# qhy991/llama.cpp-quant-gemm

Measured on NVIDIA B200. Metric: q4_0_q8_1_decode_gemv_hbm_gbs, higher is better.
Workload: dtype u4 x s8 -> s32 (dp4a), fp32 fold

## Files before the change

### llama.cpp-quant-gemm_b200/csrc/gemv.cu

```cuda
#include <cstdlib>

#include "ptx.cuh"
#include "qgemm_common.cuh"

namespace qgemm {

constexpr int kGemvWarps = 8;
constexpr int kGemvThreads = (kGemvWarps + 1) * 32;
constexpr int kGemvMaxStages = 8;
constexpr int kGemvInflightTarget = 56 * 1024;
constexpr int kGemvSlotsOff = 128;
constexpr int kGemvAbarOff = kGemvSlotsOff + 2 * kGemvWarps * 8 * 4;
constexpr int kGemvActOff = (kGemvAbarOff + 8 + 127) / 128 * 128;
static_assert(2 * kGemvMaxStages * 8 <= kGemvSlotsOff, "ring barriers overlap the slots");
static_assert(kGemvAbarOff % 8 == 0 && kGemvAbarOff + 8 <= kGemvActOff, "abar must not overlap the bulk-copy destination");
constexpr int kGemvSmemBudget = 110 * 1024;
constexpr int kGemvCtasPerSm = 2;
constexpr int kGemvMaxGroup = 8;
constexpr int kGemvTileTarget = 24 * 1024;

template <int WT> struct Pair { static constexpr int words = Fmt<WT>::bytes / 2; };

template <int WT>
__device__ __forceinline__ void load_pair(const uint8_t* p, uint32_t (&x)[Pair<WT>::words]) {
    if constexpr (WT == QGEMM_TYPE_Q5_1) {
        const uint4* q = reinterpret_cast<const uint4*>(p);
#pragma unroll
        for (int i = 0; i < 3; i++) {
            const uint4 v = q[i];
            x[4 * i] = v.x; x[4 * i + 1] = v.y; x[4 * i + 2] = v.z; x[4 * i + 3] = v.w;
        }
    } else if constexpr (WT == QGEMM_TYPE_Q4_1) {
        const uint2* q = reinterpret_cast<const uint2*>(p);
#pragma unroll
        for (int i = 0; i < 5; i++) {
            const uint2 v = q[i];
            x[2 * i] = v.x; x[2 * i + 1] = v.y;
        }
    } else {
        const uint32_t* q = reinterpret_cast<const uint32_t*>(p);
#pragma unroll
        for (int i = 0; i < Pair<WT>::words; i++) x[i] = q[i];
    }
}

__device__ __forceinline__ void expand4(const uint32_t (&q)[4], uint32_t (&w)[8]) {
#pragma unroll
    for (int i = 0; i < 4; i++) {
        w[i] = q[i] & 0x0f0f0f0fu;
        w[i + 4] = q[i] & 0xf0f0f0f0u;
    }
}
// ... 40 lines not shown
        ws[0] = {half_bits_to_float(x[0]), 0.f};
        ws[1] = {half_bits_to_float(x[5] >> 16), 0.f};
        const uint32_t q0[4] = {fs(x[1], x[2]), fs(x[2], x[3]), fs(x[3], x[4]), fs(x[4], x[5])};
        const uint32_t q1[4] = {x[7], x[8], x[9], x[10]};
        expand5(q0, fs(x[0], x[1]), w[0]);
        expand5(q1, x[6], w[1]);
    } else if constexpr (WT == QGEMM_TYPE_Q5_1) {
        ws[0] = {half_bits_to_float(x[0]), half_bits_to_float(x[0] >> 16)};
        ws[1] = {half_bits_to_float(x[6]), half_bits_to_float(x[6] >> 16)};
        const uint32_t q0[4] = {x[2], x[3], x[4], x[5]};
        const uint32_t q1[4] = {x[8], x[9], x[10], x[11]};
        expand5(q0, x[1], w[0]);
        expand5(q1, x[7], w[1]);
    } else {
        ws[0] = {half_bits_to_float(x[0]), 0.f};
        ws[1] = {half_bits_to_float(x[8] >> 16), 0.f};
#pragma unroll
        for (int i = 0; i < 8; i++) {
            w[0][i] = fs(x[i], x[i + 1]);
            w[1][i] = x[9 + i];
        }
    }
}

struct ActPair {
    int q[2][8];
    ActScale s[2];
};

struct GemvParams {
    const uint8_t* act;
    const uint8_t* wgt;
    float* C;
    int F, nb;
    int64_t ldc_t, ldc_f;
    int RT;
    int WPR;
    int stages;
    int stage_bytes;
    int pdl;
    int nocompute;
    int act_bulk;
    PeerOut peer;
    const uint8_t* pf_ptr;
    unsigned long long pf_bytes;
    int nmat;
    const uint8_t* wgt_m[kGemvMaxGroup];
    float* C_m[kGemvMaxGroup];
    int fstart[kGemvMaxGroup + 1];
    float skew;
#ifdef QGEMM_GEMV_TRACE
    int trace_slot;
#endif
};

#ifdef QGEMM_GEMV_TRACE
constexpr int kTraceSlots = 256, kTraceCtas = 304;
__device__ unsigned long long g_gemv_trace[kTraceSlots][kTraceCtas][6];
__device__ __forceinline__ unsigned long long gtimer() {
    unsigned long long t;
    asm volatile("mov.u64 %0, %%globaltimer;" : "=l"(t));
    return t;
}
#define GEMV_TRACE(i) do { if (threadIdx.x == 0 && blockIdx.x < kTraceCtas) g_gemv_trace[p.trace_slot][blockIdx.x][i] = gtimer(); } while (0)
#else
#define GEMV_TRACE(i)
#endif

struct TileRef { int m, local, rows; };
__device__ __forceinline__ TileRef tile_at(const GemvParams& p, int r0, int r_end) {
    TileRef t{0, r0, min(p.RT, r_end - r0)};
    if (p.nmat > 1) {
        int m = 0;
        while (m + 1 < p.nmat && r0 >= p.fstart[m + 1]) m++;
        t.m = m;
        t.local = r0 - p.fstart[m];
        t.rows = min(t.rows, p.fstart[m + 1] - r0);
    }
    return t;
}

template <int WT, int TT, int PPL, bool kMsExact, bool kFull>
__global__ void __launch_bounds__(kGemvThreads, kGemvCtasPerSm) gemv_kernel(const GemvParams p) {
    using Fm = Fmt<WT>;
    extern __shared__ __align__(128) uint8_t smem[];
    const int tid = threadIdx.x, warp = tid >> 5, lane = tid & 31;
    const int nb = p.nb, np = nb >> 1;

    uint64_t* full = reinterpret_cast<uint64_t*>(smem);
    uint64_t* empty = full + kGemvMaxStages;
    float* slots = reinterpret_cast<float*>(smem + kGemvSlotsOff);
    uint8_t* a_raw = smem + kGemvActOff;
    float4* a_scale = reinterpret_cast<float4*>(smem + kGemvActOff);
    uint4* a_qs = reinterpret_cast<uint4*>(smem + kGemvActOff + (size_t)TT * np * 16);
    const uint32_t act_bytes = (PPL > 0) ? (uint32_t)TT * nb * 36u : (uint32_t)TT * nb * 40u;
    uint8_t* stage0 = smem + (((uint32_t)kGemvActOff + act_bytes + 127u) & ~127u);

    auto span_at = [&](unsigned c) -> int {
        if (c >= gridDim.x) return p.F;
        const float x = (float)c / (float)gridDim.x;
        const float g = x * (1.0f + 0.5f * p.skew) - 0.5f * p.skew * x * x;
        return min(p.F, (int)((float)p.F * g + 0.5f));
    };
    const int r_begin = p.skew == 0.0f ? (int)(((int64_t)p.F * blockIdx.x) / gridDim.x) : span_at(blockIdx.x);
    const int r_end = p.skew == 0.0f ? (int)(((int64_t)p.F * (blockIdx.x + 1)) / gridDim.x) : span_at(blockIdx.x + 1);
    const size_t rowbytes = (size_t)nb * Fm::bytes;

    uint64_t* abar = reinterpret_cast<uint64_t*>(smem + kGemvAbarOff);
    if (tid == 0) {
        for (int s = 0; s < p.stages; s++) {
            ptx::mbar_init(&full[s], 1);
            ptx::mbar_init(&empty[s], kGemvWarps);
        }
        ptx::mbar_init(abar, 1);
        ptx::fence_mbar_init();
    }
    __syncthreads();
    if (p.pdl) ptx::griddep_launch_dependents();

    if (warp == kGemvWarps) {
        if (lane == 0) {
            int s = 0;
            uint32_t ph = 0;
            for (int r0 = r_begin; r0 < r_end;) {
                const TileRef tr = tile_at(p, r0, r_end);
                const uint8_t* src = (p.nmat > 1 ? p.wgt_m[tr.m] : p.wgt) + (size_t)tr.local * rowbytes;
                const uint32_t bytes = (uint32_t)(tr.rows * rowbytes);
                ptx::mbar_wait(&empty[s], ph ^ 1);
                ptx::mbar_arrive_expect_tx(&full[s], bytes);
                ptx::bulk_g2s(stage0 + (size_t)s * p.stage_bytes, src, bytes, &full[s]);
                if (++s == p.stages) { s = 0; ph ^= 1; }
                r0 += tr.rows;
            }
            if (p.pf_ptr) {
                const unsigned long long chunk = ((p.pf_bytes / gridDim.x) + 15ull) & ~15ull;
                unsigned long long off = chunk * blockIdx.x;
                const unsigned long long end = min(off + chunk, p.pf_bytes & ~15ull);
                for (; off < end; off += 16384ull)
                    ptx::bulk_prefetch_l2(p.pf_ptr + off, (uint32_t)min(16384ull, end - off));
            }
        }
        return;
    }

    GEMV_TRACE(0);
    if (p.pdl == 1) ptx::griddep_wait();
    GEMV_TRACE(1);
    if (p.peer.world > 1) {
        if (tid == 0) peer_wait_prior(p.peer);
        ptx::bar_sync(1, kGemvWarps * 32);
    }
    const int WPR = p.WPR;
    const int rpp = kGemvWarps / WPR;
    const int rslot = warp / WPR, sub = warp - rslot * WPR;

    ActPair areg[PPL > 0 ? TT : 1][PPL > 0 ? PPL : 1];
    if constexpr (PPL > 0) {
        const uint32_t* a32 = reinterpret_cast<const uint32_t*>(p.act);
        uint32_t* dst = reinterpret_cast<uint32_t*>(a_raw);
        const int total = TT * nb * 9;
        if (p.act_bulk) {
            if (tid == 0) {
                ptx::mbar_arrive_expect_tx(abar, (uint32_t)total * 4u);
                ptx::bulk_g2s(a_raw, p.act, (uint32_t)total * 4u, abar);
            }
            ptx::mbar_wait(abar, 0);
            GEMV_TRACE(4);
        } else {
            for (int i = tid; i < total; i += kGemvWarps * 32) dst[i] = __ldg(a32 + i);
            ptx::bar_sync(1, kGemvWarps * 32);
        }
#pragma unroll
        for (int j = 0; j < PPL; j++) {
            const int pg = (j * WPR + sub) * 32 + lane;
#pragma unroll
            for (int t = 0; t < TT; t++) {
                if (kFull || j < PPL - 1 || pg < np) {
                    const uint32_t* w = dst + ((size_t)t * nb + 2 * pg) * 9;
#pragma unroll
                    for (int b = 0; b < 2; b++) {
                        const uint32_t ds = w[9 * b];
                        areg[t][j].s[b] = prep_act_scale<WT, kMsExact>(half_bits_to_float(ds), half_bits_to_float(ds >> 16));
#pragma unroll
                        for (int i = 0; i < 8; i++) areg[t][j].q[b][i] = (int)w[9 * b + 1 + i];
                    }
                }
            }
        }
    } else {
        const uint32_t* a32 = reinterpret_cast<const uint32_t*>(p.act);
        float* sc = reinterpret_cast<float*>(a_scale);
        uint32_t* qs = reinterpret_cast<uint32_t*>(a_qs);
        const int total = TT * nb * 9;
        for (int i = tid; i < total; i += kGemvWarps * 32) {
            const int blk = i / 9, wd = i - blk * 9;
            const int t = blk / nb, b = blk - t * nb;
            const uint32_t v = __ldg(a32 + i);
            if (wd == 0) {
                const ActScale ps = prep_act_scale<WT, kMsExact>(half_bits_to_float(v), half_bits_to_float(v >> 16));
                float* d = sc + ((size_t)t * np + (b >> 1)) * 4 + (b & 1) * 2;
                d[0] = ps.d;
                d[1] = ps.s;
            } else {
                const int e = wd - 1;
                const int quad = (b & 1) * 2 + (e >> 2);
                qs[(((size_t)t * 4 + quad) * np + (b >> 1)) * 4 + (e & 3)] = v;
            }
        }
        ptx::bar_sync(1, kGemvWarps * 32);
    }

    GEMV_TRACE(2);
    int s = 0, spar = 0;
    uint32_t ph = 0;
    const int npl = (PPL > 0) ? PPL : (np + WPR * 32 - 1) / (WPR * 32);
    for (int g0 = r_begin; g0 < r_end;) {
        const TileRef tr = tile_at(p, g0, r_end);
        const int r0 = tr.local, rows = tr.rows;
        float* Cm = p.nmat > 1 ? p.C_m[tr.m] : p.C;
        g0 += rows;
        ptx::mbar_wait(&full[s], ph);
        const uint8_t* tile = stage0 + (size_t)s * p.stage_bytes;
        for (int pass = 0; pass * rpp < rows && !p.nocompute; pass++) {
            const int r = pass * rpp + rslot;
            float acc[TT];
#pragma unroll
            for (int tt = 0; tt < TT; tt++) acc[tt] = 0.f;
            if (r < rows) {
                const uint8_t* rowp = tile + (size_t)r * rowbytes;
                auto do_pair = [&](int j, int pg) {
                    uint32_t x[Pair<WT>::words];
                    uint32_t w[2][8];
                    WScale ws[2];
                    load_pair<WT>(rowp + (size_t)pg * (2 * Fm::bytes), x);
                    expand_pair<WT>(x, w, ws);
#pragma unroll
                    for (int tt = 0; tt < TT; tt++) {
                        if constexpr (PPL > 0) {
                            const ActPair& a = areg[tt][j];
                            acc[tt] = fold_block_pre<WT>(acc[tt], pair_sumi<WT>(w[0], a.q[0]), ws[0], a.s[0]);
                            acc[tt] = fold_block_pre<WT>(acc[tt], pair_sumi<WT>(w[1], a.q[1]), ws[1], a.s[1]);
                        } else {
                            const float4 sc = a_scale[(size_t)tt * np + pg];
                            int a0[8], a1[8];
                            const uint4 q0 = a_qs[((size_t)tt * 4 + 0) * np + pg];
                            const uint4 q1 = a_qs[((size_t)tt * 4 + 1) * np + pg];
                            const uint4 q2 = a_qs[((size_t)tt * 4 + 2) * np + pg];
                            const uint4 q3 = a_qs[((size_t)tt * 4 + 3) * np + pg];
                            a0[0] = q0.x; a0[1] = q0.y; a0[2] = q0.z; a0[3] = q0.w;
                            a0[4] = q1.x; a0[5] = q1.y; a0[6] = q1.z; a0[7] = q1.w;
                            a1[0] = q2.x; a1[1] = q2.y; a1[2] = q2.z; a1[3] = q2.w;
                            a1[4] = q3.x; a1[5] = q3.y; a1[6] = q3.z; a1[7] = q3.w;
                            acc[tt] = fold_block_pre<WT>(acc[tt], pair_sumi<WT>(w[0], a0), ws[0], ActScale{sc.x, sc.y});
                            acc[tt] = fold_block_pre<WT>(acc[tt], pair_sumi<WT>(w[1], a1), ws[1], ActScale{sc.z, sc.w});
                        }
                    }
                };
                if constexpr (PPL > 0) {
#pragma unroll
                    for (int j = 0; j < PPL; j++) {
                        const int pg = (j * WPR + sub) * 32 + lane;
                        if (kFull || j < PPL - 1 || pg < np) do_pair(j, pg);
                    }
                } else {
                    for (int j = 0; j < npl; j++) {
                        const int pg = (j * WPR + sub) * 32 + lane;
                        if (pg < np) do_pair(0, pg);
                    }
                }
            }
#pragma unroll
            for (int tt = 0; tt < TT; tt++) {
#pragma unroll
                for (int o = 16; o > 0; o >>= 1) acc[tt] += __shfl_xor_sync(0xffffffffu, acc[tt], o);
            }
            if (WPR == 1) {
                if (r < rows && lane < TT) {
                    float v = acc[0];
#pragma unroll
                    for (int tt = 1; tt < TT; tt++) v = (lane == tt) ? acc[tt] : v;
                    peer_store(p.peer, Cm, (int64_t)lane * p.ldc_t + (int64_t)(r0 + r) * p.ldc_f, v, tr.m);
                }
            } else {
                float* sl = slots + spar * (kGemvWarps * 8);
                if (lane == 0) {
#pragma unroll
                    for (int tt = 0; tt < TT; tt++) sl[warp * 8 + tt] = acc[tt];
                }
                ptx::bar_sync(2 + rslot, WPR * 32);
                if (sub == 0 && lane < TT && r < rows) {
                    float v = 0.f;
                    for (int k = 0; k < WPR; k++) v += sl[(rslot * WPR + k) * 8 + lane];
                    peer_store(p.peer, Cm, (int64_t)lane * p.ldc_t + (int64_t)(r0 + r) * p.ldc_f, v, tr.m);
                }
                spar ^= 1;
            }
        }
        __syncwarp();
        if (lane == 0) ptx::mbar_arrive(&empty[s]);
        if (++s == p.stages) { s = 0; ph ^= 1; }
    }
    GEMV_TRACE(3);
    if (p.peer.world > 1) {
        if (!(p.peer.dbg & 4)) __threadfence();
        ptx::bar_sync(1, kGemvWarps * 32);
        if (tid == 0) peer_signal_done(p.peer, gridDim.x);
    }
    if (p.pdl == 2) ptx::griddep_wait();
}

struct GemvPlan {
    int tt;
    int ppl;
    int wpr;
    int rt;
    int stages, stage_bytes;
    size_t smem;
};

static bool gemv_plan(int wtype, int T, int F, int K, int grid, bool pdl, GemvPlan* pl);

bool gemv_supported(int wtype, const void* act, const void* wgt, int F, int K) {
    const int nb = K / 32;
    const size_t rowbytes = (size_t)nb * block_bytes(wtype);
    if (F < 1 || nb < 2 || (nb & 1)) return false;
    if (rowbytes % 16 != 0 || rowbytes > 64 * 1024) return false;
    if (reinterpret_cast<uintptr_t>(wgt) % 16 != 0) return false;
    if (reinterpret_cast<uintptr_t>(act) % 4 != 0) return false;
    GemvPlan pl;
    return gemv_plan(wtype, 1, F, K, 1, false, &pl);
}

static bool gemv_plan(int wtype, int T, int F, int K, int grid, bool pdl, GemvPlan* pl) {
    const int nb = K / 32, np = nb / 2;
    const size_t rowbytes = (size_t)nb * block_bytes(wtype);
    for (int tt = min(T, 8); tt >= 1; tt--) {
        int ppl = 0, wpr = 1;
        for (int w = 1; w <= kGemvWarps; w <<= 1) {
            const int need = (np + 32 * w - 1) / (32 * w);
            if (need * tt <= 3) { ppl = need; wpr = w; break; }
        }
        if (QGEMM_ENV("QGEMM_GEMV_FORCE_SMEM")) ppl = 0;
        if (ppl == 0) {
            wpr = 1;
            while (wpr < kGemvWarps && np > 64 * wpr) wpr <<= 1;
        }
        const int rpp = kGemvWarps / wpr;
        int rt = rpp;
        while (rt < 8 && (size_t)(2 * rt) * rowbytes <= (size_t)kGemvTileTarget) rt <<= 1;
        if (const char* e = QGEMM_ENV("QGEMM_GEMV_RT")) rt = max(rpp, atoi(e) / rpp * rpp);
        const size_t fixed = kGemvActOff + (size_t)tt * nb * (ppl == 0 ? 40 : 36) + 128;
        auto stage_of = [&](int r) { return (int)(((size_t)r * rowbytes + 127) / 128 * 128); };
        while (rt > 1 && fixed + 2 * (size_t)stage_of(rt) > (size_t)kGemvSmemBudget) rt >>= 1;
        const int stage_bytes = stage_of(rt);
        if (fixed + 2 * (size_t)stage_bytes > (size_t)kGemvSmemBudget) continue;
        int stages = (int)(((size_t)kGemvSmemBudget - fixed) / stage_bytes);
        stages = max(2, min(kGemvMaxStages, stages));
        const int rows_per_cta = (F + grid - 1) / grid;
        stages = max(2, min(stages, (rows_per_cta + rt - 1) / rt));
        stages = max(2, min(stages, kGemvInflightTarget / stage_bytes));
        (void)pdl;
        if (const char* e = QGEMM_ENV("QGEMM_GEMV_STAGES")) stages = max(2, min(kGemvMaxStages, atoi(e)));
        *pl = {tt, ppl, wpr, rt, stages, stage_bytes, fixed + (size_t)stages * stage_bytes};
        return true;
    }
    return false;
}

template <int WT, int TT, int PPL>
static cudaError_t launch_gemv_inst(const GemvParams& p, size_t smem, int grid, bool ms_exact, cudaStream_t st) {
    auto launch = [&](auto kernel, int variant) -> cudaError_t {
        (void)variant;
        if (cudaError_t e = smem_optin(reinterpret_cast<const void*>(kernel), smem)) return e;
        cudaLaunchConfig_t cfg{};
        cfg.gridDim = dim3(grid);
        cfg.blockDim = dim3(kGemvThreads);
        cfg.dynamicSmemBytes = smem;
        cfg.stream = st;
        cudaLaunchAttribute at[1];
        at[0].id = cudaLaunchAttributeProgrammaticStreamSerialization;
        at[0].val.programmaticStreamSerializationAllowed = 1;
// ... 5 lines not shown
    const bool full = PPL > 0 && (p.nb / 2) == PPL * p.WPR * 32;
    if constexpr (Fmt<WT>::m >= 0) {
        if (full) e = ms_exact ? launch(gemv_kernel<WT, TT, PPL, true, true>, 2) : launch(gemv_kernel<WT, TT, PPL, false, true>, 3);
        else e = ms_exact ? launch(gemv_kernel<WT, TT, PPL, true, false>, 1) : launch(gemv_kernel<WT, TT, PPL, false, false>, 0);
    } else {
        e = full ? launch(gemv_kernel<WT, TT, PPL, false, true>, 3) : launch(gemv_kernel<WT, TT, PPL, false, false>, 0);
    }
    note_launch();
    return e;
}

template <int WT>
static cudaError_t launch_gemv_wt(const GemvPlan& pl, const GemvParams& p, int grid, bool ms, cudaStream_t st) {
#define QG_CASE(TTv, PPLv) \
    if (pl.tt == TTv && pl.ppl == PPLv) return launch_gemv_inst<WT, TTv, PPLv>(p, pl.smem, grid, ms, st);
    QG_CASE(1, 1) QG_CASE(1, 2) QG_CASE(1, 3) QG_CASE(2, 1) QG_CASE(3, 1)
    QG_CASE(1, 0) QG_CASE(2, 0) QG_CASE(3, 0) QG_CASE(4, 0) QG_CASE(5, 0) QG_CASE(6, 0) QG_CASE(7, 0) QG_CASE(8, 0)
#undef QG_CASE
    return cudaErrorInvalidValue;
}

struct GemvGroup { int nmat; const void* wgt[kGemvMaxGroup]; float* C[kGemvMaxGroup]; int F[kGemvMaxGroup]; };

cudaError_t launch_gemv(int wtype, const void* act, const void* wgt, float* C, int T, int F, int K, int64_t ldc_t,
                        int64_t ldc_f, uint32_t flags, int num_sms, cudaStream_t st, const PeerOut* peer,
                        const void* pf_ptr, size_t pf_bytes, const GemvGroup* group);

cudaError_t launch_gemv(int wtype, const void* act, const void* wgt, float* C, int T, int F, int K, int64_t ldc_t,
                        int64_t ldc_f, uint32_t flags, int num_sms, cudaStream_t st, const PeerOut* peer,
                        const void* pf_ptr, size_t pf_bytes) {
    return launch_gemv(wtype, act, wgt, C, T, F, K, ldc_t, ldc_f, flags, num_sms, st, peer, pf_ptr, pf_bytes, nullptr);
}

cudaError_t launch_gemv(int wtype, const void* act, const void* wgt, float* C, int T, int F, int K, int64_t ldc_t,
                        int64_t ldc_f, uint32_t flags, int num_sms, cudaStream_t st, const PeerOut* peer,
                        const void* pf_ptr, size_t pf_bytes, const GemvGroup* group) {
    const int nb = K / 32;
    const bool ms = flags & QGEMM_MS_EXACT;
    GemvPlan pl;
    int ctas_per_sm = kGemvCtasPerSm;
    if (const char* e = QGEMM_ENV("QGEMM_GEMV_CTAS")) ctas_per_sm = max(1, min(kGemvCtasPerSm, atoi(e)));
    const int grid = min(F, ctas_per_sm * num_sms);
    const bool pdl = flags & QGEMM_WEIGHTS_STATIC;
    if (!gemv_plan(wtype, T, F, K, grid, pdl, &pl)) return cudaErrorInvalidValue;
    for (int t0 = 0; t0 < T; t0 += pl.tt) {
        GemvPlan cur = pl;
        if (T - t0 < pl.tt && !gemv_plan(wtype, T - t0, F, K, grid, pdl, &cur)) return cudaErrorInvalidValue;
        GemvParams p;
        p.act = (const uint8_t*)act + (size_t)t0 * nb * kQ81Bytes;
        p.wgt = (const uint8_t*)wgt;
        p.C = C + (int64_t)t0 * ldc_t;
        p.F = F; p.nb = nb; p.ldc_t = ldc_t; p.ldc_f = ldc_f;
        p.RT = cur.rt; p.WPR = cur.wpr; p.stages = cur.stages; p.stage_bytes = cur.stage_bytes;
        p.pdl = pdl ? ((flags & QGEMM_INPUTS_READY) ? 2 : 1) : 0;
        p.nocompute = QGEMM_ENV("QGEMM_GEMV_NOCOMPUTE") ? 1 : 0;
        p.act_bulk = (reinterpret_cast<uintptr_t>(p.act) % 16 == 0 && ((size_t)cur.tt * nb * kQ81Bytes) % 16 == 0 &&
                      !QGEMM_ENV("QGEMM_GEMV_NO_ACT_BULK")) ? 1 : 0;
        p.pf_ptr = (t0 + pl.tt >= T && reinterpret_cast<uintptr_t>(pf_ptr) % 16 == 0) ? (const uint8_t*)pf_ptr : nullptr;
        p.pf_bytes = pf_bytes;
        p.skew = QGEMM_ENV("QGEMM_GEMV_SKEW") ? (float)atof(QGEMM_ENV("QGEMM_GEMV_SKEW")) : (F >= 8 * grid ? 0.28f : 0.0f);
#ifdef QGEMM_GEMV_TRACE
        {
            static int seq = 0;
            p.trace_slot = seq++ % kTraceSlots;
        }
#endif
        p.nmat = 0;
        if (group && group->nmat == 1) {
            p.wgt = (const uint8_t*)group->wgt[0];
            p.C = group->C[0] + (int64_t)t0 * ldc_t;
        } else if (group) {
            p.nmat = group->nmat;
            p.fstart[0] = 0;
            for (int m = 0; m < group->nmat; m++) {
                p.wgt_m[m] = (const uint8_t*)group->wgt[m];
                p.C_m[m] = group->C[m] + (int64_t)t0 * ldc_t;
                p.fstart[m + 1] = p.fstart[m] + group->F[m];
            }
        }
        p.peer = PeerOut{};
        if (peer) {
            if (T > pl.tt) return cudaErrorInvalidValue;
            p.peer = *peer;
        }
        cudaError_t e;
        switch (wtype) {
        case QGEMM_TYPE_Q4_0: e = launch_gemv_wt<QGEMM_TYPE_Q4_0>(cur, p, grid, ms, st); break;
        case QGEMM_TYPE_Q4_1: e = launch_gemv_wt<QGEMM_TYPE_Q4_1>(cur, p, grid, ms, st); break;
        case QGEMM_TYPE_Q5_0: e = launch_gemv_wt<QGEMM_TYPE_Q5_0>(cur, p, grid, ms, st); break;
        case QGEMM_TYPE_Q5_1: e = launch_gemv_wt<QGEMM_TYPE_Q5_1>(cur, p, grid, ms, st); break;
        case QGEMM_TYPE_Q8_0: e = launch_gemv_wt<QGEMM_TYPE_Q8_0>(cur, p, grid, ms, st); break;
        default: e = cudaErrorInvalidValue;
        }
        if (e != cudaSuccess) return e;
    }
    return cudaSuccess;
}


constexpr int kChainMaxSteps = 160;
constexpr int kChainMaxMat = 3;
constexpr int kChainQStride = 1536 * 36;

struct ChainStep {
    const uint8_t* act;
    const float* x;
    const float* gate;
    const uint8_t* wgt[kChainMaxMat];
    float* C[kChainMaxMat];
    int fstart[kChainMaxMat + 1];
    int nb;
    int ldc_f;
    unsigned char nmat, RT, WPR, ppl, full, wait;
};

template <int NS> struct ChainParams {
    int nsteps;
// ... 241 lines not shown
    }
}

struct ChainStepHost {
    const void* act; const float* x; const float* gate;
    int nmat; const void* wgt[kChainMaxMat]; float* C[kChainMaxMat]; int F[kChainMaxMat];
    int K; int ldc_f; int wait;
};

int gemv_chain_max_steps() { return kChainMaxSteps; }
static size_t gemv_chain_counter_bytes(int) { return ((size_t)(2 * kChainMaxSteps + 1) * sizeof(unsigned) + 255) / 256 * 256; }
size_t gemv_chain_sync_bytes(int nsteps) { return gemv_chain_counter_bytes(nsteps) + 2 * (size_t)kChainQStride; }

template <int NS>
static bool gemv_chain_plan(int wtype, const ChainStepHost* steps, int nsteps, int grid, ChainParams<NS>* out, size_t* smem) {
    if (nsteps < 1 || nsteps > NS) return false;
    int stage_bytes = 0;
    size_t act_bytes = 0;
    for (int k = 0; k < nsteps; k++) {
        const ChainStepHost& h = steps[k];
        if (h.nmat < 1 || h.nmat > kChainMaxMat) return false;
        const int nb = h.K / 32;
        int Ftot = 0;
        for (int m = 0; m < h.nmat; m++) {
            if (!gemv_supported(wtype, h.act ? h.act : (const void*)h.x, h.wgt[m], h.F[m], h.K)) return false;
            Ftot += h.F[m];
        }
        if (h.act) {
            if (reinterpret_cast<uintptr_t>(h.act) % 16 != 0 || ((size_t)nb * kQ81Bytes) % 16 != 0) return false;
        } else {
            if (reinterpret_cast<uintptr_t>(h.x) % 16 != 0 || (h.gate && reinterpret_cast<uintptr_t>(h.gate) % 16 != 0)) return false;
        }
        GemvPlan pl;
        if (!gemv_plan(wtype, 1, Ftot, h.K, grid, true, &pl) || pl.tt != 1 || pl.ppl < 1 || pl.ppl > 3) return false;
        ChainStep& st = out->st[k];
        st = ChainStep{};
        st.act = (const uint8_t*)h.act; st.x = h.x; st.gate = h.gate;
        st.fstart[0] = 0;
        for (int m = 0; m < h.nmat; m++) {
            st.wgt[m] = (const uint8_t*)h.wgt[m];
            st.C[m] = h.C[m];
            st.fstart[m + 1] = st.fstart[m] + h.F[m];
        }
        for (int m = h.nmat; m < kChainMaxMat; m++) st.fstart[m + 1] = st.fstart[h.nmat];
        st.nb = nb; st.ldc_f = h.ldc_f;
        st.nmat = (unsigned char)h.nmat; st.RT = (unsigned char)pl.rt; st.WPR = (unsigned char)pl.wpr; st.ppl = (unsigned char)pl.ppl;
        st.full = (nb / 2) == pl.ppl * pl.wpr * 32 ? 1 : 0;
        st.wait = h.wait ? 1 : 0;
        stage_bytes = max(stage_bytes, (int)(((size_t)pl.rt * nb * block_bytes(wtype) + 127) / 128 * 128));
        act_bytes = max(act_bytes, (size_t)nb * kQ81Bytes);
    }
    const size_t fixed = (((size_t)kGemvActOff + act_bytes + 127) & ~(size_t)127);
    if (fixed + 2 * (size_t)stage_bytes > (size_t)kGemvSmemBudget) return false;
    int stages = (int)(((size_t)kGemvSmemBudget - fixed) / stage_bytes);
    stages = max(2, min(kGemvMaxStages, stages));
    if (const char* e = QGEMM_ENV("QGEMM_CHAIN_STAGES")) stages = max(2, min(stages, atoi(e)));
    out->nsteps = nsteps;
    out->stages = stages;
    out->stage_bytes = stage_bytes;
    out->act_bytes = (uint32_t)act_bytes;
    *smem = fixed + (size_t)stages * stage_bytes;
    return true;
}

template <int WT, int NS>
static cudaError_t launch_chain_wt(const ChainParams<NS>& p, size_t smem, int num_sms, cudaStream_t st) {
    auto kernel = gemv_chain_kernel<WT, NS>;
// ... 62 lines not shown
```

### profiles/microbench/decode_trace.cu

```cuda
#include <algorithm>
#include <cstdint>
#include <cstdio>
#include <cstdlib>
#include <dlfcn.h>
#include <vector>
#include <cuda_runtime.h>
#include "qgemm.h"

#define CK(x) do { cudaError_t e_ = (x); if (e_ != cudaSuccess) { printf("CUDA error %s at line %d\n", cudaGetErrorString(e_), __LINE__); return 1; } } while (0)
#define QK(x) do { int r_ = (x); if (r_ != 0) { printf("qgemm error %d (%s) at line %d\n", r_, qgemm_strerror(r_), __LINE__); return 1; } } while (0)

int main() {
    typedef int (*read_fn)(unsigned long long*, size_t);
    read_fn rd = (read_fn)dlsym(RTLD_DEFAULT, "qgemm_debug_read_gemv_trace");
    if (!rd) { printf("preload a -DQGEMM_GEMV_TRACE build of the library\n"); return 2; }
    const int layers = 32, per = 7;
    const int Fs[per] = {4096, 4096, 4096, 4096, 11008, 11008, 4096}, Ks[per] = {4096, 4096, 4096, 4096, 4096, 4096, 11008};
    std::vector<size_t> off(layers * per + 1, 0);
    for (int i = 0; i < layers * per; i++) off[i + 1] = off[i] + ((size_t)Fs[i % per] * (Ks[i % per] / 32) * 18 + 255) / 256 * 256;
    uint8_t* arena; CK(cudaMalloc(&arena, off.back()));
    CK(cudaMemset(arena, 0x11, off.back()));
    uint8_t *a4k, *a11k; float* out;
    CK(cudaMalloc(&a4k, 128 * 36)); CK(cudaMalloc(&a11k, 344 * 36)); CK(cudaMalloc(&out, 4 * 11008 * sizeof(float)));
    CK(cudaMemset(a4k, 0, 128 * 36)); CK(cudaMemset(a11k, 0, 344 * 36));
// ... 9 lines not shown
            hint(b + 3);
            QK(qgemm_gemm_group(QGEMM_TYPE_Q4_0, a4k, 3, g3, c3, f3, 1, 4096, 1, 1, QGEMM_WEIGHTS_STATIC, st));
            hint(b + 4);
            QK(qgemm_gemm(QGEMM_TYPE_Q4_0, a4k, arena + off[b + 3], out, 1, 4096, 4096, 1, 1, QGEMM_WEIGHTS_STATIC, nullptr, 0, st));
            const void* g2[2] = {arena + off[b + 4], arena + off[b + 5]};
            float* c2[2] = {out, out + 11008};
            const int f2[2] = {11008, 11008};
            hint(b + 6);
            QK(qgemm_gemm_group(QGEMM_TYPE_Q4_0, a4k, 2, g2, c2, f2, 1, 4096, 1, 1, QGEMM_WEIGHTS_STATIC, st));
            hint(b + 7);
            QK(qgemm_gemm(QGEMM_TYPE_Q4_0, a11k, arena + off[b + 6], out, 1, 4096, 11008, 1, 1, QGEMM_WEIGHTS_STATIC, nullptr, 0, st));
        }
        return 0;
    };
    cudaGraph_t g; cudaGraphExec_t ge;
    CK(cudaStreamBeginCapture(st, cudaStreamCaptureModeGlobal));
    if (step()) return 1;
    CK(cudaStreamEndCapture(st, &g));
    CK(cudaGraphInstantiate(&ge, g, 0));
    cudaEvent_t e0, e1; CK(cudaEventCreate(&e0)); CK(cudaEventCreate(&e1));
    for (int r = 0; r < 3; r++) CK(cudaGraphLaunch(ge, st));
    CK(cudaEventRecord(e0, st));
    CK(cudaGraphLaunch(ge, st));
    CK(cudaEventRecord(e1, st));
    CK(cudaStreamSynchronize(st));
    float ms; CK(cudaEventElapsedTime(&ms, e0, e1));
    printf("one step (128 launches): %.1f us\n", ms * 1e3);
    const int slots = 256, ctas = 304, nl = layers * 4;
    std::vector<unsigned long long> tr((size_t)slots * ctas * 6);
    if (rd(tr.data(), tr.size() * 8)) { printf("trace read failed\n"); return 1; }
    auto T = [&](int l, int c, int i) { return tr[((size_t)(l % slots) * ctas + c) * 6 + i]; };
    const int grid = 296;
    double sum_wait2bulk = 0, sum_wait2bulk_mean = 0, sum_gap = 0, sum_skew = 0, sum_startskew = 0, sum_wait2act = 0, sum_len = 0, sum_period = 0;
    int cnt = 0;
    unsigned long long t0 = ~0ull;
    for (int c = 0; c < grid; c++) t0 = std::min(t0, T(0, c, 0));
    for (int l = 0; l < nl; l++) {
        unsigned long long s_min = ~0ull, s_max = 0, w_min = ~0ull, w_max = 0, a_max = 0, e_min = ~0ull, e_max = 0;
        for (int c = 0; c < grid; c++) {
            s_min = std::min(s_min, T(l, c, 0)); s_max = std::max(s_max, T(l, c, 0));
            w_min = std::min(w_min, T(l, c, 1)); w_max = std::max(w_max, T(l, c, 1));
            a_max = std::max(a_max, T(l, c, 2));
            e_min = std::min(e_min, T(l, c, 3)); e_max = std::max(e_max, T(l, c, 3));
        }
        if (l >= 8 && l < 24)
            printf("launch %3d (%s): first CTA in %7.2f  last CTA in %7.2f | wait passed %7.2f .. %7.2f | acts ready (last) %7.2f | first CTA done %7.2f  last CTA done %7.2f us\n",
                   l, (const char*[]){"qkv", "wo ", "g/u", "dwn"}[l % 4], (s_min - t0) * 1e-3, (s_max - t0) * 1e-3, (w_min - t0) * 1e-3, (w_max - t0) * 1e-3,
                   (a_max - t0) * 1e-3, (e_min - t0) * 1e-3, (e_max - t0) * 1e-3);
        if (l >= 4 && l + 1 < nl) {
            unsigned long long nw_min = ~0ull, ne_max = 0;
            for (int c = 0; c < grid; c++) { nw_min = std::min(nw_min, T(l + 1, c, 1)); ne_max = std::max(ne_max, T(l + 1, c, 3)); }
            sum_gap += (double)nw_min - (double)e_max;
            sum_skew += (double)e_max - (double)e_min;
            sum_startskew += (double)w_max - (double)w_min;
            sum_wait2act += (double)a_max - (double)w_max;
            { unsigned long long b_max = 0; double m = 0; for (int c = 0; c < grid; c++) { b_max = std::max(b_max, T(l, c, 4)); m += (double)T(l, c, 4) - (double)T(l, c, 1); } sum_wait2bulk += (double)b_max - (double)w_max; sum_wait2bulk_mean += m / grid; }
            sum_len += (double)e_max - (double)w_min;
            sum_period += (double)ne_max - (double)e_max;
            cnt++;
        }
    }
    for (int l = 8; l < 12; l++) {
        std::vector<std::pair<unsigned long long, unsigned long long>> se;
        for (int c = 0; c < grid; c++) se.push_back({T(l, c, 0), T(l, c, 3)});
        std::sort(se.begin(), se.end());
        double q[4] = {0, 0, 0, 0};
        for (int c = 0; c < grid; c++) q[c * 4 / grid] += (double)(se[c].second - t0) * 1e-3 / (grid / 4);
        int lo = 0, hi = 0;
        double elo = 0, ehi = 0;
        for (int c = 0; c < grid; c++) { if (c < grid / 2) { elo += (double)(T(l, c, 3) - t0) * 1e-3; lo++; } else { ehi += (double)(T(l, c, 3) - t0) * 1e-3; hi++; } }
        printf("launch %d: mean end time by start-time quartile (earliest starters first): %.2f %.2f %.2f %.2f us | by block index half: %.2f %.2f\n", l, q[0], q[1], q[2], q[3],
               elo / lo, ehi / hi);
    }
    printf("wait passed -> activation bulk copy complete: last CTA %.2f us, mean over CTAs %.2f us\n", sum_wait2bulk / cnt * 1e-3, sum_wait2bulk_mean / cnt * 1e-3);
    printf("averages over %d launches (us): period %.2f | wait passed -> last store %.2f | last store -> next launch past its wait %.2f | "
           "skew of the waits %.2f | last wait -> activations in registers %.2f | skew of the last stores %.2f\n",
           cnt, sum_period / cnt * 1e-3, sum_len / cnt * 1e-3, sum_gap / cnt * 1e-3, sum_startskew / cnt * 1e-3, sum_wait2act / cnt * 1e-3, sum_skew / cnt * 1e-3);
    return 0;
}
```

Before: 4255.

## Replace static per-CTA row spans with atomic dynamic chunk claiming in GEMV

Each CTA's producer lane now claims weight-row chunks from a global atomic counter instead of processing a fixed, skew-shaped contiguous span. The chunk to process is passed to the consumer warps through a small shared-memory descriptor ring. The tail of the last matrix is split into half-size chunks so CTAs finish closer together. The goal is to cut end-of-kernel straggler skew, at the cost of one atomic per chunk, a per-launch counter slot with last-CTA reset logic, and a loss of contiguous per-CTA streaming.

```diff
diff --git a/llama.cpp-quant-gemm_b200/csrc/gemv.cu b/llama.cpp-quant-gemm_b200/csrc/gemv.cu
--- a/llama.cpp-quant-gemm_b200/csrc/gemv.cu
+++ b/llama.cpp-quant-gemm_b200/csrc/gemv.cu
@@ -1,3 +1,4 @@
+#include <atomic>
 #include <cstdlib>
 
 #include "ptx.cuh"
@@ -11,13 +12,21 @@
 constexpr int kGemvInflightTarget = 56 * 1024;
 constexpr int kGemvSlotsOff = 128;
 constexpr int kGemvAbarOff = kGemvSlotsOff + 2 * kGemvWarps * 8 * 4;
-constexpr int kGemvActOff = (kGemvAbarOff + 8 + 127) / 128 * 128;
+constexpr int kGemvDescOff = kGemvAbarOff + 8;
+constexpr int kGemvActOff = (kGemvDescOff + 8 * kGemvMaxStages + 127) / 128 * 128;
 static_assert(2 * kGemvMaxStages * 8 <= kGemvSlotsOff, "ring barriers overlap the slots");
-static_assert(kGemvAbarOff % 8 == 0 && kGemvAbarOff + 8 <= kGemvActOff, "abar must not overlap the bulk-copy destination");
+static_assert(kGemvAbarOff % 8 == 0 && kGemvDescOff + 8 * kGemvMaxStages <= kGemvActOff,
+              "abar / descriptors must not overlap the bulk-copy destination");
 constexpr int kGemvSmemBudget = 110 * 1024;
 constexpr int kGemvCtasPerSm = 2;
 constexpr int kGemvMaxGroup = 8;
 constexpr int kGemvTileTarget = 24 * 1024;
+constexpr int kGemvMaxSegs = kGemvMaxGroup + 1;
+
+constexpr int kGemvEagerSlots = 1024, kGemvGraphSlots = 15360;
+__device__ unsigned g_gemv_claims[kGemvEagerSlots + kGemvGraphSlots][2];
+
+struct GemvSeg { int c0, m, r0, r1, rows; };
 
 template <int WT> struct Pair { static constexpr int words = Fmt<WT>::bytes / 2; };
 
@@ -124,7 +133,7 @@
     const uint8_t* act;
     const uint8_t* wgt;
     float* C;
-    int F, nb;
+    int nb;
     int64_t ldc_t, ldc_f;
     int RT;
     int WPR;
@@ -139,8 +148,9 @@
     int nmat;
     const uint8_t* wgt_m[kGemvMaxGroup];
     float* C_m[kGemvMaxGroup];
-    int fstart[kGemvMaxGroup + 1];
-    float skew;
+    unsigned* claim;
+    int nchunks, nseg;
+    GemvSeg seg[kGemvMaxSegs];
 #ifdef QGEMM_GEMV_TRACE
     int trace_slot;
 #endif
@@ -159,17 +169,11 @@
 #define GEMV_TRACE(i)
 #endif
 
-struct TileRef { int m, local, rows; };
-__device__ __forceinline__ TileRef tile_at(const GemvParams& p, int r0, int r_end) {
-    TileRef t{0, r0, min(p.RT, r_end - r0)};
-    if (p.nmat > 1) {
-        int m = 0;
-        while (m + 1 < p.nmat && r0 >= p.fstart[m + 1]) m++;
-        t.m = m;
-        t.local = r0 - p.fstart[m];
-        t.rows = min(t.rows, p.fstart[m + 1] - r0);
-    }
-    return t;
+__device__ __forceinline__ int2 chunk_at(const GemvParams& p, int c) {
+    int i = 0;
+    while (i + 1 < p.nseg && c >= p.seg[i + 1].c0) i++;
+    const int r0 = p.seg[i].r0 + (c - p.seg[i].c0) * p.seg[i].rows;
+    return make_int2(r0, (p.seg[i].m << 16) | min(p.seg[i].rows, p.seg[i].r1 - r0));
 }
 
 template <int WT, int TT, int PPL, bool kMsExact, bool kFull>
@@ -187,15 +191,7 @@
     uint4* a_qs = reinterpret_cast<uint4*>(smem + kGemvActOff + (size_t)TT * np * 16);
     const uint32_t act_bytes = (PPL > 0) ? (uint32_t)TT * nb * 36u : (uint32_t)TT * nb * 40u;
     uint8_t* stage0 = smem + (((uint32_t)kGemvActOff + act_bytes + 127u) & ~127u);
-
-    auto span_at = [&](unsigned c) -> int {
-        if (c >= gridDim.x) return p.F;
-        const float x = (float)c / (float)gridDim.x;
-        const float g = x * (1.0f + 0.5f * p.skew) - 0.5f * p.skew * x * x;
-        return min(p.F, (int)((float)p.F * g + 0.5f));
-    };
-    const int r_begin = p.skew == 0.0f ? (int)(((int64_t)p.F * blockIdx.x) / gridDim.x) : span_at(blockIdx.x);
-    const int r_end = p.skew == 0.0f ? (int)(((int64_t)p.F * (blockIdx.x + 1)) / gridDim.x) : span_at(blockIdx.x + 1);
+    int2* desc = reinterpret_cast<int2*>(smem + kGemvDescOff);
     const size_t rowbytes = (size_t)nb * Fm::bytes;
 
     uint64_t* abar = reinterpret_cast<uint64_t*>(smem + kGemvAbarOff);
@@ -214,15 +210,30 @@
         if (lane == 0) {
             int s = 0;
             uint32_t ph = 0;
-            for (int r0 = r_begin; r0 < r_end;) {
-                const TileRef tr = tile_at(p, r0, r_end);
-                const uint8_t* src = (p.nmat > 1 ? p.wgt_m[tr.m] : p.wgt) + (size_t)tr.local * rowbytes;
-                const uint32_t bytes = (uint32_t)(tr.rows * rowbytes);
+            int c = (int)atomicAdd(p.claim, 1u);
+            for (;;) {
+                const bool more = c < p.nchunks;
+                const int c_next = more ? (int)atomicAdd(p.claim, 1u) : c;
                 ptx::mbar_wait(&empty[s], ph ^ 1);
+                if (!more) {
+                    desc[s] = make_int2(0, 0);
+                    ptx::mbar_arrive(&full[s]);
+                    break;
+                }
+                const int2 d = chunk_at(p, c);
+                const int m = d.y >> 16, rows = d.y & 0xffff;
+                const uint8_t* src = (p.nmat > 1 ? p.wgt_m[m] : p.wgt) + (size_t)d.x * rowbytes;
+                const uint32_t bytes = (uint32_t)(rows * rowbytes);
+                desc[s] = d;
                 ptx::mbar_arrive_expect_tx(&full[s], bytes);
                 ptx::bulk_g2s(stage0 + (size_t)s * p.stage_bytes, src, bytes, &full[s]);
                 if (++s == p.stages) { s = 0; ph ^= 1; }
-                r0 += tr.rows;
+                c = c_next;
+            }
+            __threadfence();
+            if (atomicAdd(p.claim + 1, 1u) == gridDim.x - 1) {
+                p.claim[0] = 0u;
+                p.claim[1] = 0u;
             }
             if (p.pf_ptr) {
                 const unsigned long long chunk = ((p.pf_bytes / gridDim.x) + 15ull) & ~15ull;
@@ -306,12 +317,12 @@
     int s = 0, spar = 0;
     uint32_t ph = 0;
     const int npl = (PPL > 0) ? PPL : (np + WPR * 32 - 1) / (WPR * 32);
-    for (int g0 = r_begin; g0 < r_end;) {
-        const TileRef tr = tile_at(p, g0, r_end);
-        const int r0 = tr.local, rows = tr.rows;
-        float* Cm = p.nmat > 1 ? p.C_m[tr.m] : p.C;
-        g0 += rows;
+    for (;;) {
         ptx::mbar_wait(&full[s], ph);
+        const int2 d = desc[s];
+        const int r0 = d.x, rows = d.y & 0xffff, tm = d.y >> 16;
+        if (rows == 0) break;
+        float* Cm = p.nmat > 1 ? p.C_m[tm] : p.C;
         const uint8_t* tile = stage0 + (size_t)s * p.stage_bytes;
         for (int pass = 0; pass * rpp < rows && !p.nocompute; pass++) {
             const int r = pass * rpp + rslot;
@@ -371,7 +382,7 @@
                     float v = acc[0];
 #pragma unroll
                     for (int tt = 1; tt < TT; tt++) v = (lane == tt) ? acc[tt] : v;
-                    peer_store(p.peer, Cm, (int64_t)lane * p.ldc_t + (int64_t)(r0 + r) * p.ldc_f, v, tr.m);
+                    peer_store(p.peer, Cm, (int64_t)lane * p.ldc_t + (int64_t)(r0 + r) * p.ldc_f, v, tm);
                 }
             } else {
                 float* sl = slots + spar * (kGemvWarps * 8);
@@ -383,7 +394,7 @@
                 if (sub == 0 && lane < TT && r < rows) {
                     float v = 0.f;
                     for (int k = 0; k < WPR; k++) v += sl[(rslot * WPR + k) * 8 + lane];
-                    peer_store(p.peer, Cm, (int64_t)lane * p.ldc_t + (int64_t)(r0 + r) * p.ldc_f, v, tr.m);
+                    peer_store(p.peer, Cm, (int64_t)lane * p.ldc_t + (int64_t)(r0 + r) * p.ldc_f, v, tm);
                 }
                 spar ^= 1;
             }
@@ -510,6 +521,49 @@
     return launch_gemv(wtype, act, wgt, C, T, F, K, ldc_t, ldc_f, flags, num_sms, st, peer, pf_ptr, pf_bytes, nullptr);
 }
 
+static void gemv_chunks(GemvParams& p, const GemvGroup* group, int F, int grid) {
+    const int nmat = group ? group->nmat : 1;
+    const int half = max(1, p.RT / 2);
+    const int F_last = group ? group->F[nmat - 1] : F;
+    const int tail = p.RT > 1 ? min(F_last, grid * half) : 0;
+    p.nseg = 0;
+    p.nchunks = 0;
+    auto add = [&](int m, int r0, int r1, int rows) {
+        if (r1 <= r0) return;
+        p.seg[p.nseg++] = GemvSeg{p.nchunks, m, r0, r1, rows};
+        p.nchunks += (r1 - r0 + rows - 1) / rows;
+    };
+    for (int m = 0; m < nmat; m++) {
+        const int Fm = group ? group->F[m] : F;
+        add(m, 0, Fm - (m == nmat - 1 ? tail : 0), p.RT);
+    }
+    add(nmat - 1, F_last - tail, F_last, half);
+}
+
+static cudaError_t gemv_claim_slot(cudaStream_t st, unsigned** slot) {
+    static std::atomic<unsigned> eager_seq{0}, graph_seq{0};
+    static std::atomic<unsigned*> base[64];
+    int dev = 0;
+    if (cudaError_t e = cudaGetDevice(&dev)) return e;
+    if (dev < 0 || dev >= 64) return cudaErrorInvalidDevice;
+    unsigned* b = base[dev].load(std::memory_order_acquire);
+    if (!b) {
+        void* a = nullptr;
+        if (cudaError_t e = cudaGetSymbolAddress(&a, g_gemv_claims)) return e;
+        b = static_cast<unsigned*>(a);
+        base[dev].store(b, std::memory_order_release);
+    }
+    cudaStreamCaptureStatus cs = cudaStreamCaptureStatusNone;
+    if (cudaStreamIsCapturing(st, &cs) != cudaSuccess) {
+        (void)cudaGetLastError();
+        cs = cudaStreamCaptureStatusNone;
+    }
+    const unsigned i = cs == cudaStreamCaptureStatusActive ? kGemvEagerSlots + graph_seq++ % kGemvGraphSlots
+                                                           : eager_seq++ % kGemvEagerSlots;
+    *slot = b + 2 * i;
+    return cudaSuccess;
+}
+
 cudaError_t launch_gemv(int wtype, const void* act, const void* wgt, float* C, int T, int F, int K, int64_t ldc_t,
                         int64_t ldc_f, uint32_t flags, int num_sms, cudaStream_t st, const PeerOut* peer,
                         const void* pf_ptr, size_t pf_bytes, const GemvGroup* group) {
@@ -528,7 +582,7 @@
         p.act = (const uint8_t*)act + (size_t)t0 * nb * kQ81Bytes;
         p.wgt = (const uint8_t*)wgt;
         p.C = C + (int64_t)t0 * ldc_t;
-        p.F = F; p.nb = nb; p.ldc_t = ldc_t; p.ldc_f = ldc_f;
+        p.nb = nb; p.ldc_t = ldc_t; p.ldc_f = ldc_f;
         p.RT = cur.rt; p.WPR = cur.wpr; p.stages = cur.stages; p.stage_bytes = cur.stage_bytes;
         p.pdl = pdl ? ((flags & QGEMM_INPUTS_READY) ? 2 : 1) : 0;
         p.nocompute = QGEMM_ENV("QGEMM_GEMV_NOCOMPUTE") ? 1 : 0;
@@ -536,7 +590,6 @@
                       !QGEMM_ENV("QGEMM_GEMV_NO_ACT_BULK")) ? 1 : 0;
         p.pf_ptr = (t0 + pl.tt >= T && reinterpret_cast<uintptr_t>(pf_ptr) % 16 == 0) ? (const uint8_t*)pf_ptr : nullptr;
         p.pf_bytes = pf_bytes;
-        p.skew = QGEMM_ENV("QGEMM_GEMV_SKEW") ? (float)atof(QGEMM_ENV("QGEMM_GEMV_SKEW")) : (F >= 8 * grid ? 0.28f : 0.0f);
 #ifdef QGEMM_GEMV_TRACE
         {
             static int seq = 0;
@@ -549,18 +602,18 @@
             p.C = group->C[0] + (int64_t)t0 * ldc_t;
         } else if (group) {
             p.nmat = group->nmat;
-            p.fstart[0] = 0;
             for (int m = 0; m < group->nmat; m++) {
                 p.wgt_m[m] = (const uint8_t*)group->wgt[m];
                 p.C_m[m] = group->C[m] + (int64_t)t0 * ldc_t;
-                p.fstart[m + 1] = p.fstart[m] + group->F[m];
-            }
-        }
+            }
+        }
+        gemv_chunks(p, group && group->nmat > 1 ? group : nullptr, F, grid);
         p.peer = PeerOut{};
         if (peer) {
             if (T > pl.tt) return cudaErrorInvalidValue;
             p.peer = *peer;
         }
+        if (cudaError_t e = gemv_claim_slot(st, &p.claim)) return e;
         cudaError_t e;
         switch (wtype) {
         case QGEMM_TYPE_Q4_0: e = launch_gemv_wt<QGEMM_TYPE_Q4_0>(cur, p, grid, ms, st); break;
diff --git a/profiles/microbench/decode_trace.cu b/profiles/microbench/decode_trace.cu
--- a/profiles/microbench/decode_trace.cu
+++ b/profiles/microbench/decode_trace.cu
@@ -65,6 +65,8 @@
     auto T = [&](int l, int c, int i) { return tr[((size_t)(l % slots) * ctas + c) * 6 + i]; };
     const int grid = 296;
     double sum_wait2bulk = 0, sum_wait2bulk_mean = 0, sum_gap = 0, sum_skew = 0, sum_startskew = 0, sum_wait2act = 0, sum_len = 0, sum_period = 0;
+    double type_spread[4] = {0, 0, 0, 0}, type_period[4] = {0, 0, 0, 0};
+    int type_n[4] = {0, 0, 0, 0}, type_np[4] = {0, 0, 0, 0};
     int cnt = 0;
     unsigned long long t0 = ~0ull;
     for (int c = 0; c < grid; c++) t0 = std::min(t0, T(0, c, 0));
@@ -90,6 +92,10 @@
             { unsigned long long b_max = 0; double m = 0; for (int c = 0; c < grid; c++) { b_max = std::max(b_max, T(l, c, 4)); m += (double)T(l, c, 4) - (double)T(l, c, 1); } sum_wait2bulk += (double)b_max - (double)w_max; sum_wait2bulk_mean += m / grid; }
             sum_len += (double)e_max - (double)w_min;
             sum_period += (double)ne_max - (double)e_max;
+            type_spread[l % 4] += (double)e_max - (double)e_min;
+            type_n[l % 4]++;
+            type_period[(l + 1) % 4] += (double)ne_max - (double)e_max;
+            type_np[(l + 1) % 4]++;
             cnt++;
         }
     }
@@ -109,5 +115,9 @@
     printf("averages over %d launches (us): period %.2f | wait passed -> last store %.2f | last store -> next launch past its wait %.2f | "
            "skew of the waits %.2f | last wait -> activations in registers %.2f | skew of the last stores %.2f\n",
            cnt, sum_period / cnt * 1e-3, sum_len / cnt * 1e-3, sum_gap / cnt * 1e-3, sum_startskew / cnt * 1e-3, sum_wait2act / cnt * 1e-3, sum_skew / cnt * 1e-3);
+    printf("by launch type (us): first CTA done -> last CTA done | period ending with this launch\n");
+    for (int k = 0; k < 4; k++)
+        printf("  %s  %.2f | %.2f\n", (const char*[]){"qkv", "wo ", "g/u", "dwn"}[k], type_spread[k] / type_n[k] * 1e-3,
+               type_period[k] / type_np[k] * 1e-3);
     return 0;
 }
```

Measured after the change: 4153, median of 6. -2.4%, worse.

## Process multiple rows per warp in GEMV consumer to amortize activation reuse

Applied to the files above, without the earlier changes.

Each consumer warp now handles R rows per pass (4 when one pair per lane, 2 for ppl=2, T=1), loading all R weight rows before expanding and dotting them against the register-resident activations. The warp reductions are interleaved across rows, and the lanes store the R outputs in parallel. The goal is to raise memory-level parallelism and cut the per-row overhead of reductions and stores in the drain-bound consumer. The tile row target grows to match, and the chain path keeps one row per warp. A profiling script that separates the consumer's time from the copy pipeline is also added.

```diff
diff --git a/llama.cpp-quant-gemm_b200/csrc/gemv.cu b/llama.cpp-quant-gemm_b200/csrc/gemv.cu
--- a/llama.cpp-quant-gemm_b200/csrc/gemv.cu
+++ b/llama.cpp-quant-gemm_b200/csrc/gemv.cu
@@ -18,6 +18,12 @@
 constexpr int kGemvCtasPerSm = 2;
 constexpr int kGemvMaxGroup = 8;
 constexpr int kGemvTileTarget = 24 * 1024;
+
+__host__ __device__ constexpr int gemv_rows_per_warp(int wt, int tt, int ppl) {
+    return (tt != 1 || ppl == 0 || (wt == QGEMM_TYPE_Q5_1 && ppl == 3)) ? 1 : (ppl == 1 ? 4 : 2);
+}
+template <int N> struct IntC { static constexpr int value = N; };
+static_assert(gemv_rows_per_warp(QGEMM_TYPE_Q4_0, 1, 1) <= 8, "a warp's outputs must fit its 8 slots");
 
 template <int WT> struct Pair { static constexpr int words = Fmt<WT>::bytes / 2; };
 
@@ -245,6 +251,8 @@
     const int WPR = p.WPR;
     const int rpp = kGemvWarps / WPR;
     const int rslot = warp / WPR, sub = warp - rslot * WPR;
+    constexpr int R = gemv_rows_per_warp(WT, TT, PPL);
+    const int rpw = rpp * R;
 
     ActPair areg[PPL > 0 ? TT : 1][PPL > 0 ? PPL : 1];
     if constexpr (PPL > 0) {
@@ -313,25 +321,24 @@
         g0 += rows;
         ptx::mbar_wait(&full[s], ph);
         const uint8_t* tile = stage0 + (size_t)s * p.stage_bytes;
-        for (int pass = 0; pass * rpp < rows && !p.nocompute; pass++) {
-            const int r = pass * rpp + rslot;
-            float acc[TT];
-#pragma unroll
-            for (int tt = 0; tt < TT; tt++) acc[tt] = 0.f;
-            if (r < rows) {
-                const uint8_t* rowp = tile + (size_t)r * rowbytes;
-                auto do_pair = [&](int j, int pg) {
-                    uint32_t x[Pair<WT>::words];
+        auto dot_rows = [&](auto nr_c, const int rfirst, float (&a)[decltype(nr_c)::value][TT]) {
+            constexpr int NR = decltype(nr_c)::value;
+            auto do_pair = [&](int j, int pg) {
+                uint32_t x[NR][Pair<WT>::words];
+#pragma unroll
+                for (int k = 0; k < NR; k++)
+                    load_pair<WT>(tile + (size_t)(rfirst + k * rpp) * rowbytes + (size_t)pg * (2 * Fm::bytes), x[k]);
+#pragma unroll
+                for (int k = 0; k < NR; k++) {
                     uint32_t w[2][8];
                     WScale ws[2];
-                    load_pair<WT>(rowp + (size_t)pg * (2 * Fm::bytes), x);
-                    expand_pair<WT>(x, w, ws);
+                    expand_pair<WT>(x[k], w, ws);
 #pragma unroll
                     for (int tt = 0; tt < TT; tt++) {
                         if constexpr (PPL > 0) {
-                            const ActPair& a = areg[tt][j];
-                            acc[tt] = fold_block_pre<WT>(acc[tt], pair_sumi<WT>(w[0], a.q[0]), ws[0], a.s[0]);
-                            acc[tt] = fold_block_pre<WT>(acc[tt], pair_sumi<WT>(w[1], a.q[1]), ws[1], a.s[1]);
+                            const ActPair& ap = areg[tt][j];
+                            a[k][tt] = fold_block_pre<WT>(a[k][tt], pair_sumi<WT>(w[0], ap.q[0]), ws[0], ap.s[0]);
+                            a[k][tt] = fold_block_pre<WT>(a[k][tt], pair_sumi<WT>(w[1], ap.q[1]), ws[1], ap.s[1]);
                         } else {
                             const float4 sc = a_scale[(size_t)tt * np + pg];
                             int a0[8], a1[8];
@@ -343,47 +350,76 @@
                             a0[4] = q1.x; a0[5] = q1.y; a0[6] = q1.z; a0[7] = q1.w;
                             a1[0] = q2.x; a1[1] = q2.y; a1[2] = q2.z; a1[3] = q2.w;
                             a1[4] = q3.x; a1[5] = q3.y; a1[6] = q3.z; a1[7] = q3.w;
-                            acc[tt] = fold_block_pre<WT>(acc[tt], pair_sumi<WT>(w[0], a0), ws[0], ActScale{sc.x, sc.y});
-                            acc[tt] = fold_block_pre<WT>(acc[tt], pair_sumi<WT>(w[1], a1), ws[1], ActScale{sc.z, sc.w});
+                            a[k][tt] = fold_block_pre<WT>(a[k][tt], pair_sumi<WT>(w[0], a0), ws[0], ActScale{sc.x, sc.y});
+                            a[k][tt] = fold_block_pre<WT>(a[k][tt], pair_sumi<WT>(w[1], a1), ws[1], ActScale{sc.z, sc.w});
                         }
                     }
-                };
-                if constexpr (PPL > 0) {
-#pragma unroll
-                    for (int j = 0; j < PPL; j++) {
-                        const int pg = (j * WPR + sub) * 32 + lane;
-                        if (kFull || j < PPL - 1 || pg < np) do_pair(j, pg);
-                    }
-                } else {
-                    for (int j = 0; j < npl; j++) {
-                        const int pg = (j * WPR + sub) * 32 + lane;
-                        if (pg < np) do_pair(0, pg);
+                }
+            };
+            if constexpr (PPL > 0) {
+#pragma unroll
+                for (int j = 0; j < PPL; j++) {
+                    const int pg = (j * WPR + sub) * 32 + lane;
+                    if (kFull || j < PPL - 1 || pg < np) do_pair(j, pg);
+                }
+            } else {
+                for (int j = 0; j < npl; j++) {
+                    const int pg = (j * WPR + sub) * 32 + lane;
+                    if (pg < np) do_pair(0, pg);
+                }
+            }
+        };
+        for (int pass = 0; pass * rpw < rows && !p.nocompute; pass++) {
+            const int rb = pass * rpw + rslot;
+            float acc[R][TT];
+#pragma unroll
+            for (int k = 0; k < R; k++) {
+#pragma unroll
+                for (int tt = 0; tt < TT; tt++) acc[k][tt] = 0.f;
+            }
+            if (rb + (R - 1) * rpp < rows) {
+                dot_rows(IntC<R>{}, rb, acc);
+            } else {
+                for (int k = 0; k < R - 1 && rb + k * rpp < rows; k++) {
+                    float a1[1][TT];
+#pragma unroll
+                    for (int tt = 0; tt < TT; tt++) a1[0][tt] = 0.f;
+                    dot_rows(IntC<1>{}, rb + k * rpp, a1);
+#pragma unroll
+                    for (int kk = 0; kk < R; kk++) {
+                        if (kk == k) {
+#pragma unroll
+                            for (int tt = 0; tt < TT; tt++) acc[kk][tt] = a1[0][tt];
+                        }
                     }
                 }
             }
 #pragma unroll
-            for (int tt = 0; tt < TT; tt++) {
-#pragma unroll
-                for (int o = 16; o > 0; o >>= 1) acc[tt] += __shfl_xor_sync(0xffffffffu, acc[tt], o);
-            }
+            for (int o = 16; o > 0; o >>= 1) {
+#pragma unroll
+                for (int k = 0; k < R; k++) {
+#pragma unroll
+                    for (int tt = 0; tt < TT; tt++) acc[k][tt] += __shfl_xor_sync(0xffffffffu, acc[k][tt], o);
+                }
+            }
+            float v = acc[0][0];
+#pragma unroll
+            for (int k = 0; k < R; k++) {
+#pragma unroll
+                for (int tt = 0; tt < TT; tt++) v = (lane == k * TT + tt) ? acc[k][tt] : v;
+            }
+            const int ko = TT == 1 ? lane : 0, to = TT == 1 ? 0 : lane, ro = rb + ko * rpp;
             if (WPR == 1) {
-                if (r < rows && lane < TT) {
-                    float v = acc[0];
-#pragma unroll
-                    for (int tt = 1; tt < TT; tt++) v = (lane == tt) ? acc[tt] : v;
-                    peer_store(p.peer, Cm, (int64_t)lane * p.ldc_t + (int64_t)(r0 + r) * p.ldc_f, v, tr.m);
-                }
+                if (lane < R * TT && ro < rows)
+                    peer_store(p.peer, Cm, (int64_t)to * p.ldc_t + (int64_t)(r0 + ro) * p.ldc_f, v, tr.m);
             } else {
                 float* sl = slots + spar * (kGemvWarps * 8);
-                if (lane == 0) {
-#pragma unroll
-                    for (int tt = 0; tt < TT; tt++) sl[warp * 8 + tt] = acc[tt];
-                }
+                if (lane < R * TT) sl[warp * 8 + lane] = v;
                 ptx::bar_sync(2 + rslot, WPR * 32);
-                if (sub == 0 && lane < TT && r < rows) {
-                    float v = 0.f;
-                    for (int k = 0; k < WPR; k++) v += sl[(rslot * WPR + k) * 8 + lane];
-                    peer_store(p.peer, Cm, (int64_t)lane * p.ldc_t + (int64_t)(r0 + r) * p.ldc_f, v, tr.m);
+                if (sub == 0 && lane < R * TT && ro < rows) {
+                    float s = 0.f;
+                    for (int k = 0; k < WPR; k++) s += sl[(rslot * WPR + k) * 8 + lane];
+                    peer_store(p.peer, Cm, (int64_t)to * p.ldc_t + (int64_t)(r0 + ro) * p.ldc_f, s, tr.m);
                 }
                 spar ^= 1;
             }
@@ -410,7 +446,7 @@
     size_t smem;
 };
 
-static bool gemv_plan(int wtype, int T, int F, int K, int grid, bool pdl, GemvPlan* pl);
+static bool gemv_plan(int wtype, int T, int F, int K, int grid, bool pdl, GemvPlan* pl, bool one_row_per_warp = false);
 
 bool gemv_supported(int wtype, const void* act, const void* wgt, int F, int K) {
     const int nb = K / 32;
@@ -423,7 +459,7 @@
     return gemv_plan(wtype, 1, F, K, 1, false, &pl);
 }
 
-static bool gemv_plan(int wtype, int T, int F, int K, int grid, bool pdl, GemvPlan* pl) {
+static bool gemv_plan(int wtype, int T, int F, int K, int grid, bool pdl, GemvPlan* pl, bool one_row_per_warp) {
     const int nb = K / 32, np = nb / 2;
     const size_t rowbytes = (size_t)nb * block_bytes(wtype);
     for (int tt = min(T, 8); tt >= 1; tt--) {
@@ -438,7 +474,7 @@
             while (wpr < kGemvWarps && np > 64 * wpr) wpr <<= 1;
         }
         const int rpp = kGemvWarps / wpr;
-        int rt = rpp;
+        int rt = rpp * (one_row_per_warp ? 1 : gemv_rows_per_warp(wtype, tt, ppl));
         while (rt < 8 && (size_t)(2 * rt) * rowbytes <= (size_t)kGemvTileTarget) rt <<= 1;
         if (const char* e = QGEMM_ENV("QGEMM_GEMV_RT")) rt = max(rpp, atoi(e) / rpp * rpp);
         const size_t fixed = kGemvActOff + (size_t)tt * nb * (ppl == 0 ? 40 : 36) + 128;
@@ -868,7 +904,7 @@
             if (reinterpret_cast<uintptr_t>(h.x) % 16 != 0 || (h.gate && reinterpret_cast<uintptr_t>(h.gate) % 16 != 0)) return false;
         }
         GemvPlan pl;
-        if (!gemv_plan(wtype, 1, Ftot, h.K, grid, true, &pl) || pl.tt != 1 || pl.ppl < 1 || pl.ppl > 3) return false;
+        if (!gemv_plan(wtype, 1, Ftot, h.K, grid, true, &pl, true) || pl.tt != 1 || pl.ppl < 1 || pl.ppl > 3) return false;
         ChainStep& st = out->st[k];
         st = ChainStep{};
         st.act = (const uint8_t*)h.act; st.x = h.x; st.gate = h.gate;
diff --git a/profiles/drain_probe.py b/profiles/drain_probe.py
--- /dev/null
+++ b/profiles/drain_probe.py
@@ -0,0 +1,82 @@
+import argparse
+import json
+import os
+import subprocess
+import sys
+
+ROOT = os.path.dirname(os.path.dirname(os.path.abspath(__file__)))
+SHAPES = ((4096, 4096), (11008, 4096))
+
+
+def child(lib_path, launches, reps):
+    sys.path[:0] = [os.path.join(ROOT, "llama.cpp-quant-gemm_b200"), ROOT]
+    import torch
+    import bench_detail
+    from quant_gemm import _lib
+    _lib.LIB_PATH = lib_path
+    import quant_gemm
+    dev = torch.device("cuda", 0)
+    out = []
+    for F, K in SHAPES:
+        w = bench_detail.make_weights(torch, 2, F, K, 1, dev, seed=7)[0]
+        aq = quant_gemm.quantize_q8_1(torch.randn((1, K), device=dev))
+        c = torch.empty((F, 1), device=dev)
+        stream = torch.cuda.Stream()
+        with torch.cuda.stream(stream):
+            quant_gemm.gemm(w, aq, F, 1, K, 2, 0x10, out=c)
+            stream.synchronize()
+            g = torch.cuda.CUDAGraph()
+            with torch.cuda.graph(g, stream=stream):
+                for _ in range(launches):
+                    quant_gemm.gemm(w, aq, F, 1, K, 2, 0x10, out=c)
+            for _ in range(3):
+                g.replay()
+            best = 1e30
+            for _ in range(reps):
+                e0, e1 = torch.cuda.Event(enable_timing=True), torch.cuda.Event(enable_timing=True)
+                e0.record(stream)
+                g.replay()
+                e1.record(stream)
+                stream.synchronize()
+                best = min(best, e0.elapsed_time(e1) * 1e3 / launches)
+        out.append({"F": F, "K": K, "us": best})
+    print(json.dumps(out))
+
+
+def main():
+    ap = argparse.ArgumentParser()
+    ap.add_argument("--lib", action="append", default=[], help="NAME=PATH of a libqgemm_sm100.so (repeatable)")
+    ap.add_argument("--launches", type=int, default=400)
+    ap.add_argument("--reps", type=int, default=10)
+    ap.add_argument("--json", default=None)
+    ap.add_argument("--child", default=None, help=argparse.SUPPRESS)
+    args = ap.parse_args()
+    if args.child:
+        return child(args.child, args.launches, args.reps)
+    libs = [tuple(s.split("=", 1)) for s in args.lib] or [
+        ("repo", os.path.join(ROOT, "llama.cpp-quant-gemm_b200", "lib", "libqgemm_sm100.so"))]
+    rows = []
+    for name, path in libs:
+        res = {}
+        for mode in ("math", "nocompute"):
+            env = dict(os.environ)
+            env.pop("QGEMM_GEMV_NOCOMPUTE", None)
+            if mode == "nocompute":
+                env["QGEMM_GEMV_NOCOMPUTE"] = "1"
+            cmd = [sys.executable, os.path.abspath(__file__), "--child", os.path.abspath(path),
+                   "--launches", str(args.launches), "--reps", str(args.reps)]
+            res[mode] = json.loads(subprocess.check_output(cmd, env=env).decode().strip().splitlines()[-1])
+        for a, b in zip(res["math"], res["nocompute"]):
+            rows.append({"lib": name, "F": a["F"], "K": a["K"], "us_math": round(a["us"], 3),
+                         "us_nocompute": round(b["us"], 3), "us_consumer": round(a["us"] - b["us"], 3)})
+    print(f"{'lib':>8} {'F x K':>12} {'math us':>9} {'nocompute us':>13} {'consumer us':>12}")
+    for r in rows:
+        print(f"{r['lib']:>8} {str(r['F']) + 'x' + str(r['K']):>12} {r['us_math']:>9.3f} {r['us_nocompute']:>13.3f} "
+              f"{r['us_consumer']:>12.3f}")
+    if args.json:
+        with open(args.json, "w") as f:
+            json.dump(rows, f, indent=1)
+
+
+if __name__ == "__main__":
+    main()
```

Result: faster. 4240 before, 4423 after (median of 6 runs) (+4.3%).
